# XiSHEN0220/RANSAC-Flow

Measured on NVIDIA H100. Metric: image-pairs/sec at 480x640, nbIter=1k RANSAC, higher is better.
Workload: dtype f32-grade: fp16 hi/lo split operands and activations (22 significand bits), 3 wgmma MMAs per MAC, fp32 accumulate; fp16-split correlation; fp32/fp64 RANSAC

## Files before the change

ransac-flow_b200/csrc/gemm_tc.cu:

```cuda
#include <cuda.h>
#include <cuda_fp16.h>

#include <climits>
#include <mutex>
#include <unordered_map>

#include "common.cuh"
#include "tc_common.cuh"

namespace rf {

constexpr int K_TF32 = 0, K_F16 = 1, K_SPLIT = 2, K_TF32X3 = 3;
constexpr int MODE_CONV = 0, MODE_CORR = 1;
constexpr int O_F32 = 0, O_F16 = 1, O_SPLIT = 2;
constexpr int WG_THREADS = 288;

struct alignas(64) WgParams {
    CUtensorMap mapA[RF_MAX_IMGS];
    CUtensorMap mapA2[RF_MAX_IMGS];
    CUtensorMap mapY[RF_MAX_IMGS];
    CUtensorMap mapR[RF_MAX_IMGS];
    CUtensorMap mapB;
    CUtensorMap mapBlo;
    int nimg;
    int ntiles;
    int tile_start[RF_MAX_IMGS + 1];
    int tiles_x[RF_MAX_IMGS];
    int tw[RF_MAX_IMGS];
    int Ho[RF_MAX_IMGS], Wo[RF_MAX_IMGS];
    long long out_pix[RF_MAX_IMGS + 1];
    int R, S, pad, stride, Cin, Cout, relu, round_out;
    int dil;
    int kc1, stride2;
    long long plane;
    const float* bias;
    const void* residual;
    void* y;
    unsigned long long* rowbest;
    unsigned long long* colbest;
    int NA, NB;
};
static_assert(sizeof(WgParams) <= 32764, "kernel parameter space (CUDA 12.1+ large kernel parameters)");

template <int KIND, int BN, int MODE>
struct WgCfg {
    static constexpr int NPL = (KIND == K_SPLIT || KIND == K_TF32X3) ? 2 : 1;
    static constexpr int A_BYTES = NPL * TC_A_BYTES;
    static constexpr int B_PLANE = BN * 128;
    static constexpr int STAGE_BYTES = A_BYTES + NPL * B_PLANE;
    static constexpr bool ONE_CTA = MODE == MODE_CORR || NPL * BN >= 256;
    static constexpr int BUDGET = ONE_CTA ? 200 * 1024 : 100 * 1024;
    static constexpr int STAGES = BUDGET / STAGE_BYTES > 6 ? 6 : BUDGET / STAGE_BYTES;
    static constexpr int CTAS_PER_SM = ONE_CTA ? 1 : 2;
    static constexpr int SMEM_BYTES = STAGES * STAGE_BYTES + 1024  + 256 ;
    static_assert(STAGES >= 2 && SMEM_BYTES <= 227 * 1024, "shared memory");
};

__device__ __forceinline__ __half2 pack_sat(float a, float b) {
    uint32_t r;
    asm("cvt.rn.satfinite.f16x2.f32 %0, %1, %2;" : "=r"(r) : "f"(b), "f"(a));
    return *reinterpret_cast<__half2*>(&r);
}
__device__ __forceinline__ void split2(float a, float b, __half2& hi, __half2& lo) {
    hi = pack_sat(a, b);
    const float2 f = __half22float2(hi);
    lo = pack_sat((a - f.x) * 2048.f, (b - f.y) * 2048.f);
}

template <int KIND, int BN, int NACC>
__device__ __forceinline__ void mma_block(float (&acc)[NACC][BN / 2], uint32_t sa, uint32_t sb) {
    constexpr bool TF32 = KIND == K_TF32 || KIND == K_TF32X3;
#pragma unroll
    for (int k = 0; k < 4; ++k) {
        const uint64_t ah = wg_desc(sa + 32 * k), bh = wg_desc(sb + 32 * k);
        if constexpr (KIND == K_SPLIT || KIND == K_TF32X3) {
            const uint64_t al = wg_desc(sa + TC_A_BYTES + 32 * k), bl = wg_desc(sb + BN * 128 + 32 * k);
            float (&x)[BN / 2] = acc[NACC - 1];
            wgmma<TF32, BN>(x, al, bh);
            wgmma<TF32, BN>(x, ah, bl);
            wgmma<TF32, BN>(acc[0], ah, bh);
        } else {
            wgmma<TF32, BN>(acc[0], ah, bh);
        }
    }
}

template <int KIND, int BN, int MODE, int OUT>
__global__ void __launch_bounds__(WG_THREADS, WgCfg<KIND, BN, MODE>::CTAS_PER_SM)
wg_kernel(const __grid_constant__ WgParams p) {
    using Cfg = WgCfg<KIND, BN, MODE>;
    constexpr int STAGES = Cfg::STAGES;
    constexpr int BK = (KIND == K_TF32 || KIND == K_TF32X3) ? TC_BK : TC_BK_F16;
    constexpr int NACC = KIND == K_SPLIT ? 2 : 1;
    constexpr bool SLOT = MODE == MODE_CONV && OUT != O_F32;
    constexpr int BOX_BYTES = (OUT == O_SPLIT ? 2 : 1) * 128 * 128;
    static_assert(!SLOT || (BN / 64) * BOX_BYTES <= Cfg::STAGE_BYTES, "the output tile fits one stage");
    extern __shared__ uint8_t smem_raw[];
    uint8_t* smem = smem_raw + ((1024u - (smem_u32(smem_raw) & 1023u)) & 1023u);
    uint64_t* full = reinterpret_cast<uint64_t*>(smem + STAGES * Cfg::STAGE_BYTES);
    uint64_t* empty = full + STAGES;
    const int warp = threadIdx.x >> 5, lane = threadIdx.x & 31;
    const int kc = p.Cin / BK;
    const int KI = p.R * p.S * kc;

    const int t_first = MODE == MODE_CORR ? 0 : (int)blockIdx.x;
    const int t_step = MODE == MODE_CORR ? 1 : (int)gridDim.x;
    const int t_end = MODE == MODE_CORR ? 1 : p.ntiles;
    const int nt = (p.Cout + BN - 1) / BN;
    struct Tile { int img, tw, ox0, oy0, n0; };
    auto decode = [&](int t) {
        const int mtile = MODE == MODE_CORR ? (int)blockIdx.y : t / nt;
        const int ntile = MODE == MODE_CORR ? (int)blockIdx.x : t - mtile * nt;
        Tile T;
        T.img = 0;
#pragma unroll
        for (int j = 1; j < RF_MAX_IMGS; ++j) T.img += (j < p.nimg && mtile >= p.tile_start[j]) ? 1 : 0;
        const int tloc = mtile - p.tile_start[T.img];
        T.tw = p.tw[T.img];
        const int tyi = tloc / p.tiles_x[T.img], txi = tloc - tyi * p.tiles_x[T.img];
        T.ox0 = txi * T.tw;
        T.oy0 = tyi * (128 / T.tw);
        T.n0 = ntile * BN;
        return T;
    };
    auto boxes = [&](const Tile& T) { return BN == 64 || T.n0 + 64 >= p.Cout ? 1 : 2; };

    if (threadIdx.x == 0) {
        for (int s = 0; s < STAGES; ++s) { mbar_init(&full[s], 1); mbar_init(&empty[s], 256); }
        fence_barrier_init();
    }
    __syncthreads();

    if (warp == 8) {
        if (lane == 0) {
            tma_prefetch_desc(&p.mapB);
            uint32_t prefetched = 0;
            int st = 0;
            uint32_t ph = 0;
            for (int t = t_first; t < t_end; t += t_step) {
                const Tile T = decode(t);
                if (!((prefetched >> T.img) & 1u)) {
                    prefetched |= 1u << T.img;
                    tma_prefetch_desc(&p.mapA[T.img]);
                    if constexpr (SLOT) {
                        tma_prefetch_desc(&p.mapY[T.img]);
                        if (p.residual) tma_prefetch_desc(&p.mapR[T.img]);
                    }
                }
                for (int it = 0; it < KI; ++it) {
                    mbar_wait(&empty[st], ph ^ 1);
                    uint8_t* sa = smem + st * Cfg::STAGE_BYTES;
                    uint8_t* sb = sa + Cfg::A_BYTES;
                    mbar_expect_tx(&full[st], Cfg::STAGE_BYTES);
                    if constexpr (MODE == MODE_CORR) {
                        const int c0 = it * BK;
                        tma_load_3d(sa, &p.mapA[0], &full[st], c0, T.ox0, 0);
                        tma_load_3d(sa + TC_A_BYTES, &p.mapA2[0], &full[st], c0, T.ox0, 0);
                        tma_load_2d(sb, &p.mapB, &full[st], c0, T.n0);
                        tma_load_2d(sb + Cfg::B_PLANE, &p.mapBlo, &full[st], c0, T.n0);
                    } else {
                        const int tap = it / kc, cc = it - tap * kc;
                        const int r = tap / p.S, s = tap - r * p.S;
                        const int c0 = cc * BK, x = T.ox0 * p.stride + s * p.dil - p.pad, y = T.oy0 * p.stride + r * p.dil - p.pad;
                        const int kcol = tap * p.Cin + c0;
                        if constexpr (KIND == K_SPLIT) {
                            if (cc < p.kc1) tma_load_4d(sa, &p.mapA[T.img], &full[st], c0, x, y, 0);
                            else tma_load_4d(sa, &p.mapA2[T.img], &full[st], (cc - p.kc1) * BK, T.ox0 * p.stride2, T.oy0 * p.stride2, 0);
                            tma_load_3d(sb, &p.mapB, &full[st], kcol, T.n0, 0);
                        } else {
                            tma_load_3d(sa, &p.mapA[T.img], &full[st], c0, x, y);
                            tma_load_2d(sb, &p.mapB, &full[st], kcol, T.n0);
                        }
                    }
                    if (++st == STAGES) { st = 0; ph ^= 1; }
                }
                if constexpr (SLOT) {
                    mbar_wait(&empty[st], ph ^ 1);
                    if (p.residual) {
// ... 6 lines not shown
                        }
                    } else {
                        mbar_arrive(&full[st]);
                    }
                    if (++st == STAGES) { st = 0; ph ^= 1; }
                }
            }
        }
        return;
    }

    const int g = warp >> 2;
    const int rbase = 64 * g + 16 * (warp & 3) + (lane >> 2);
    const int cbase = 2 * (lane & 3);
    auto before = [](int s) { return s == 0 ? STAGES - 1 : s - 1; };
    int st = 0;
    uint32_t ph = 0;
    bool stored = false;
    for (int t = t_first; t < t_end; t += t_step) {
        const Tile T = decode(t);
        float acc[NACC][BN / 2];
#pragma unroll
        for (int a = 0; a < NACC; ++a)
#pragma unroll
            for (int i = 0; i < BN / 2; ++i) acc[a][i] = 0.f;
        for (int it = 0; it < KI; ++it) {
            mbar_wait(&full[st], ph);
            const uint32_t sa = smem_u32(smem + st * Cfg::STAGE_BYTES);
            wg_fence();
            mma_block<KIND, BN, NACC>(acc, sa + g * (64 * 128), sa + Cfg::A_BYTES);
            wg_commit();
            wg_wait<1>();
            if (it > 0) {
                mbar_arrive(&empty[before(st)]);
            } else if (SLOT && stored) {
                if (threadIdx.x == 0) bulk_wait_read();
                mbar_arrive(&empty[before(st)]);
            }
            if (++st == STAGES) { st = 0; ph ^= 1; }
        }
        wg_wait<0>();
#pragma unroll
        for (int a = 0; a < NACC; ++a) wg_fence_regs(acc[a]);
        mbar_arrive(&empty[before(st)]);

        auto value = [&](int i) -> float {
            if constexpr (KIND == K_SPLIT) return fmaf(acc[1][i], 0.00048828125f, acc[0][i]);
            else return acc[0][i];
        };

        if constexpr (SLOT) {
            mbar_wait(&full[st], ph);
            uint8_t* slot = smem + st * Cfg::STAGE_BYTES;
#pragma unroll
            for (int h = 0; h < 2; ++h) {
                const int m = rbase + 8 * h;
#pragma unroll
                for (int j = 0; j < BN / 8; ++j) {
                    const int c = 8 * j + cbase, n = T.n0 + c;
                    if (n >= p.Cout) continue;
                    float v0 = value(4 * j + 2 * h), v1 = value(4 * j + 2 * h + 1);
                    if (p.bias) { v0 += __ldg(p.bias + n); v1 += __ldg(p.bias + n + 1); }
                    uint8_t* e = slot + (c >> 6) * BOX_BYTES + m * 128 + ((((c & 63) >> 3) ^ (m & 7)) << 4) + (c & 7) * 2;
                    if (p.residual) {
                        if constexpr (OUT == O_F16) {
                            const float2 r = __half22float2(*reinterpret_cast<const __half2*>(e));
                            v0 += r.x; v1 += r.y;
                        } else {
                            const float2 rh = __half22float2(*reinterpret_cast<const __half2*>(e));
                            const float2 rl = __half22float2(*reinterpret_cast<const __half2*>(e + 128 * 128));
                            v0 += fmaf(rl.x, 0.00048828125f, rh.x); v1 += fmaf(rl.y, 0.00048828125f, rh.y);
                        }
                    }
                    if (p.relu) { v0 = fmaxf(v0, 0.f); v1 = fmaxf(v1, 0.f); }
                    if constexpr (OUT == O_F16) {
                        *reinterpret_cast<__half2*>(e) = pack_sat(v0, v1);
                    } else {
                        __half2 hi, lo;
                        split2(v0, v1, hi, lo);
                        *reinterpret_cast<__half2*>(e) = hi;
                        *reinterpret_cast<__half2*>(e + 128 * 128) = lo;
                    }
                }
            }
            fence_proxy_async();
            asm volatile("bar.sync 1, 256;" ::: "memory");
            if (threadIdx.x == 0) {
                const int nb = boxes(T);
                for (int b = 0; b < nb; ++b) {
                    if constexpr (OUT == O_SPLIT) tma_store_4d(&p.mapY[T.img], slot + b * BOX_BYTES, T.n0 + 64 * b, T.ox0, T.oy0, 0);
                    else tma_store_3d(&p.mapY[T.img], slot + b * BOX_BYTES, T.n0 + 64 * b, T.ox0, T.oy0);
                }
                bulk_commit();
            }
            stored = true;
            if (++st == STAGES) { st = 0; ph ^= 1; }
        } else if constexpr (MODE == MODE_CONV) {
            const int img = T.img, tw = T.tw;
#pragma unroll
            for (int h = 0; h < 2; ++h) {
                const int m = rbase + 8 * h;
                const int py = m / tw, px = m - py * tw;
                const int oy = T.oy0 + py, ox = T.ox0 + px;
                if (oy >= p.Ho[img] || ox >= p.Wo[img]) continue;
                const long long pix = p.out_pix[img] + (long long)oy * p.Wo[img] + ox;
#pragma unroll
                for (int j = 0; j < BN / 8; ++j) {
                    const int n = T.n0 + 8 * j + cbase;
                    if (n >= p.Cout) continue;
                    const bool two = n + 1 < p.Cout;
                    float v0 = value(4 * j + 2 * h), v1 = value(4 * j + 2 * h + 1);
                    if (p.bias) { v0 += __ldg(p.bias + n); if (two) v1 += __ldg(p.bias + n + 1); }
                    const long long o = pix * p.Cout + n;
                    if (p.residual) {
                        const float* r = static_cast<const float*>(p.residual) + o;
                        v0 += __ldg(r); if (two) v1 += __ldg(r + 1);
                    }
                    if (p.relu) { v0 = fmaxf(v0, 0.f); v1 = fmaxf(v1, 0.f); }
                    if (p.round_out) { v0 = round_tf32(v0); v1 = round_tf32(v1); }
                    float* y = static_cast<float*>(p.y) + o;
                    if (two && (p.Cout & 1) == 0) *reinterpret_cast<float2*>(y) = make_float2(v0, v1);
                    else { y[0] = v0; if (two) y[1] = v1; }
                }
            }
        } else {
            const int n0 = T.n0;
            unsigned long long* sCol = reinterpret_cast<unsigned long long*>(smem);
            const int row0 = T.ox0 + rbase, row1 = row0 + 8;
            const bool rv0 = row0 < p.NA, rv1 = row1 < p.NA;
            unsigned long long rb0 = 0ull, rb1 = 0ull;
            asm volatile("bar.sync 1, 256;" ::: "memory");
#pragma unroll
            for (int j = 0; j < BN / 8; ++j) {
#pragma unroll
                for (int e = 0; e < 2; ++e) {
                    const int c = 8 * j + cbase + e, col = n0 + c;
                    const bool cv = col < p.NB;
                    const float s0 = value(4 * j + e), s1 = value(4 * j + 2 + e);
                    unsigned long long ck = 0ull;
                    if (cv) {
                        if (rv0) { const unsigned long long k = pack_key(s0, (uint32_t)col); rb0 = k > rb0 ? k : rb0; ck = pack_key(s0, (uint32_t)row0); }
                        if (rv1) { const unsigned long long k = pack_key(s1, (uint32_t)col); rb1 = k > rb1 ? k : rb1;
                                   const unsigned long long k1 = pack_key(s1, (uint32_t)row1); ck = k1 > ck ? k1 : ck; }
                    }
#pragma unroll
                    for (int off = 4; off < 32; off <<= 1) {
                        const unsigned long long o = __shfl_xor_sync(0xffffffffu, ck, off);
                        ck = o > ck ? o : ck;
                    }
                    if (lane < 4) sCol[warp * BN + c] = ck;
                }
            }
#pragma unroll
            for (int off = 1; off < 4; off <<= 1) {
                const unsigned long long o0 = __shfl_xor_sync(0xffffffffu, rb0, off), o1 = __shfl_xor_sync(0xffffffffu, rb1, off);
                rb0 = o0 > rb0 ? o0 : rb0;
                rb1 = o1 > rb1 ? o1 : rb1;
            }
            if ((lane & 3) == 0) {
                if (rv0 && rb0 != 0ull) atomicMax(p.rowbest + row0, rb0);
                if (rv1 && rb1 != 0ull) atomicMax(p.rowbest + row1, rb1);
            }
            asm volatile("bar.sync 1, 256;" ::: "memory");
            for (int c = threadIdx.x; c < BN; c += 256) {
                if (n0 + c >= p.NB) continue;
                unsigned long long cb = 0ull;
#pragma unroll
                for (int w = 0; w < 8; ++w) { const unsigned long long k = sCol[w * BN + c]; cb = k > cb ? k : cb; }
                if (cb != 0ull) atomicMax(p.colbest + n0 + c, cb);
            }
        }
    }
    if constexpr (SLOT)
        if (threadIdx.x == 0) bulk_wait();
}


constexpr int ST_TW = 32, ST_TH = 4, ST_C = 3;
constexpr int ST_PW = (ST_TW - 2) / 2, ST_PH = ST_TH / 2;
constexpr int ST_THREADS = 256;
constexpr int ST_B_PLANE = 64 * 128;
constexpr int ST_T_BYTES = 128 * 64 * 4;
static_assert(ST_PH * ST_PW * 8 <= ST_THREADS, "one thread per (pooled pixel, 8 channels) of a step");

template <int KS, int S>
struct StemGeo {
    static constexpr int PAD = (KS - 1) / 2;
    static constexpr int KK = KS * KS * ST_C;
    static constexpr int KSTEPS = (KK + 15) / 16;
    static constexpr int KB = (KSTEPS + 3) / 4;
    static constexpr int IN_H = (ST_TH - 1) * S + KS;
    static constexpr int IN_COLS = (ST_TW - 1) * S + KS;
    static constexpr int IN_W = IN_COLS * ST_C;
    static constexpr int EVEN_W = (IN_COLS + 1) / 2 * ST_C;
    static constexpr int LD = S == 2 ? 208 : 104;
    static constexpr int WIN = IN_H * LD;
    static constexpr int NLD = (IN_H * IN_W + ST_THREADS - 1) / ST_THREADS;
    static constexpr int NT = S == 2 ? 3 : 2;
    static constexpr int CTAS = S == 2 ? 1 : 2;
    static constexpr int OFF_T = KB * 2 * ST_B_PLANE;
    static constexpr int OFF_IN = OFF_T + NT * ST_T_BYTES;
    static constexpr int OFF_K = OFF_IN + 2 * WIN * 4;
    static constexpr int OFF_BAR = OFF_K + KSTEPS * 4 * 16;
    static constexpr int SMEM = OFF_BAR + 64 + 1024;
    static_assert(LD >= (S == 2 ? EVEN_W + IN_COLS / 2 * ST_C : IN_W), "window row");
    static_assert(CTAS * SMEM <= 227 * 1024, "stem shared memory");
    static __device__ __forceinline__ int word(int r, int ix, int c) { return r * LD + (S == 2 ? (ix & 1) * EVEN_W + (ix >> 1) * ST_C : ix * ST_C) + c; }
};

struct alignas(64) StemParams {
    CUtensorMap mapB;
    int nimg, pool;
    int unit_start[RF_MAX_IMGS + 1];
    int steps[RF_MAX_IMGS];
    int H[RF_MAX_IMGS], W[RF_MAX_IMGS];
    int Hs[RF_MAX_IMGS], Ws[RF_MAX_IMGS];
    int Ho[RF_MAX_IMGS], Wo[RF_MAX_IMGS];
    long long in_pix[RF_MAX_IMGS], out_pix[RF_MAX_IMGS];
    long long plane;
    const float* x;
    const float* bias;
    __half* y;
};

__device__ __forceinline__ uint32_t stem_pack_split(float v) {
    __half2 hi, lo;
    split2(v, 0.f, hi, lo);
    return (*reinterpret_cast<uint32_t*>(&hi) & 0xFFFFu) | (*reinterpret_cast<uint32_t*>(&lo) << 16);
}

struct StemFrag { uint32_t h[4], l[4]; };

template <int KK, int j>
__device__ __forceinline__ void stem_gather(StemFrag& f, const uint32_t* __restrict__ w, int base, const int4* sK, int q) {
    const int4 o4 = sK[j * 4 + q];
    const int o[4] = {o4.x, o4.y, o4.z, o4.w};
    uint32_t v[2][4];
#pragma unroll
    for (int h = 0; h < 2; ++h)
#pragma unroll
        for (int e = 0; e < 4; ++e) v[h][e] = (16 * (j + 1) <= KK || o[e] >= 0) ? w[base + 24 * h + o[e]] : 0u;
#pragma unroll
    for (int e = 0; e < 2; ++e)
#pragma unroll
        for (int h = 0; h < 2; ++h) {
            f.h[2 * e + h] = __byte_perm(v[h][2 * e], v[h][2 * e + 1], 0x5410);
            f.l[2 * e + h] = __byte_perm(v[h][2 * e], v[h][2 * e + 1], 0x7632);
        }
}

template <int KK, int KSTEPS, bool SPLIT, int j, int NACC>
__device__ __forceinline__ void stem_mma(float (&acc)[NACC][32], StemFrag (&buf)[2], const uint32_t* w, int base, const int4* sK, int q,
                                         uint32_t sB) {
    if constexpr (j < KSTEPS) {
        constexpr int NPL = SPLIT ? 2 : 1;
        StemFrag& f = buf[j & 1];
        wg_fence();
        const uint32_t b = sB + (j >> 2) * NPL * ST_B_PLANE + 32 * (j & 3);
        const uint64_t bh = wg_desc(b);
        if constexpr (SPLIT) {
            wgmma_f16_n64_rs(acc[1], f.l, bh);
            wgmma_f16_n64_rs(acc[1], f.h, wg_desc(b + ST_B_PLANE));
        }
        wgmma_f16_n64_rs(acc[0], f.h, bh);
        wg_commit();
        if constexpr (j + 1 < KSTEPS) {
            wg_wait<1>();
            stem_gather<KK, j + 1>(buf[(j + 1) & 1], w, base, sK, q);
        }
        stem_mma<KK, KSTEPS, SPLIT, j + 1>(acc, buf, w, base, sK, q, sB);
    }
}

template <int KS, int S, bool SPLIT>
__global__ void __launch_bounds__(ST_THREADS, StemGeo<KS, S>::CTAS)
stem_kernel(const __grid_constant__ StemParams p) {
    using G = StemGeo<KS, S>;
    constexpr int NPL = SPLIT ? 2 : 1;
    constexpr int NACC = SPLIT ? 2 : 1;
    constexpr int PIX_BYTES = SPLIT ? 256 : 128;
    extern __shared__ uint8_t smem_raw[];
    uint8_t* smem = smem_raw + ((1024u - (smem_u32(smem_raw) & 1023u)) & 1023u);
    uint8_t* sB = smem;
    uint8_t* sT = smem + G::OFF_T;
    uint32_t* sIn = reinterpret_cast<uint32_t*>(smem + G::OFF_IN);
    int4* sK = reinterpret_cast<int4*>(smem + G::OFF_K);
    uint64_t* bar_b = reinterpret_cast<uint64_t*>(smem + G::OFF_BAR);
    const int t = threadIdx.x, warp = t >> 5, lane = t & 31, g = warp >> 2;
    const long long units = p.unit_start[RF_MAX_IMGS];
    const int u_begin = (int)(units * blockIdx.x / gridDim.x), u_end = (int)(units * (blockIdx.x + 1) / gridDim.x);

    struct Unit { int img, strip, j, r0, c0; };
    auto decode = [&](int u) {
        Unit U;
        U.img = 0;
#pragma unroll
        for (int i = 1; i < RF_MAX_IMGS; ++i) U.img += (i < p.nimg && u >= p.unit_start[i]) ? 1 : 0;
        const int loc = u - p.unit_start[U.img];
        U.strip = loc / p.steps[U.img];
        U.j = loc - U.strip * p.steps[U.img];
        U.r0 = U.j * ST_TH;
        U.c0 = p.pool ? U.strip * 2 * ST_PW - 1 : U.strip * ST_TW;
        return U;
    };
    float win[G::NLD];
    auto load_window = [&](const Unit& U) {
        const int H = p.H[U.img], WC = p.W[U.img] * ST_C;
        const float* src = p.x + p.in_pix[U.img] * ST_C;
        const int iy0 = U.r0 * S - G::PAD, col0 = (U.c0 * S - G::PAD) * ST_C;
// ... 7 lines not shown
    };
    auto stage_window = [&](uint32_t* dst) {
#pragma unroll
        for (int i = 0; i < G::NLD; ++i) {
            const int idx = t + i * ST_THREADS;
            const int r = idx / G::IN_W, jj = idx - r * G::IN_W, ix = jj / ST_C;
            if (idx < G::IN_H * G::IN_W) dst[G::word(r, ix, jj - ix * ST_C)] = stem_pack_split(win[i]);
        }
    };

    if (t == 0) {
        mbar_init(bar_b, 1);
        fence_barrier_init();
    }
    if (t < G::KSTEPS * 4) {
        const int j = t >> 2, q = t & 3;
        int o[4];
#pragma unroll
        for (int e = 0; e < 4; ++e) {
            const int k = 16 * j + 2 * q + (e & 1) + 8 * (e >> 1);
            const int r = k / (KS * ST_C), rs = k - r * KS * ST_C, s = rs / ST_C;
            o[e] = k < G::KK ? G::word(r, s, rs - s * ST_C) : -1;
        }
        sK[t] = make_int4(o[0], o[1], o[2], o[3]);
    }
    __syncthreads();
    if (t == 0) {
        mbar_expect_tx(bar_b, G::KB * NPL * ST_B_PLANE);
#pragma unroll
        for (int kb = 0; kb < G::KB; ++kb) {
            if constexpr (SPLIT) tma_load_3d(sB + kb * 2 * ST_B_PLANE, &p.mapB, bar_b, kb * 64, 0, 0);
            else tma_load_2d(sB + kb * ST_B_PLANE, &p.mapB, bar_b, kb * 64, 0);
        }
    }
    int u = u_begin;
    Unit U = decode(u);
    if (p.pool && U.j > 0) U = decode(--u);
    load_window(U);
    stage_window(sIn);
    __syncthreads();

    const int q = lane & 3;
    const int rbase = 64 * g + 16 * (warp & 3) + (lane >> 2), cbase = 2 * q;
    const int base = (rbase >> 5) * S * G::LD + 3 * (rbase & 31);
    const uint32_t sB32 = smem_u32(sB);
    int wb = 0, tb = 0;
    for (bool first = true; u < u_end; ++u, first = false) {
        const uint32_t* w = sIn + wb * G::WIN;
        float acc[NACC][32];
#pragma unroll
        for (int a = 0; a < NACC; ++a)
#pragma unroll
            for (int i = 0; i < 32; ++i) acc[a][i] = 0.f;
        StemFrag frag[2];
        stem_gather<G::KK, 0>(frag[0], w, base, sK, q);
        if (first) mbar_wait(bar_b, 0);
        stem_mma<G::KK, G::KSTEPS, SPLIT, 0>(acc, frag, w, base, sK, q, sB32);
        const bool more = u + 1 < u_end;
        Unit N = U;
        if (more) {
            N = decode(u + 1);
            load_window(N);
        }
        wg_wait<0>();
#pragma unroll
        for (int a = 0; a < NACC; ++a) wg_fence_regs(acc[a]);

        const int img = U.img;
        uint8_t* tile = sT + tb * ST_T_BYTES;
#pragma unroll
        for (int h = 0; h < 2; ++h) {
            const int mm = rbase + 8 * h;
#pragma unroll
            for (int j = 0; j < 8; ++j) {
                const int n = 8 * j + cbase, i = 4 * j + 2 * h;
                float v0 = SPLIT ? fmaf(acc[NACC - 1][i], 0.00048828125f, acc[0][i]) : acc[0][i];
                float v1 = SPLIT ? fmaf(acc[NACC - 1][i + 1], 0.00048828125f, acc[0][i + 1]) : acc[0][i + 1];
                if (p.bias) { v0 += __ldg(p.bias + n); v1 += __ldg(p.bias + n + 1); }
                v0 = fmaxf(v0, 0.f);
                v1 = fmaxf(v1, 0.f);
                uint8_t* e = tile + mm * 128 + ((j ^ (mm & 7)) << 4) + cbase * 2;
                if constexpr (SPLIT) {
                    __half2 hi, lo;
                    split2(v0, v1, hi, lo);
                    if (p.pool) {
                        const float2 fh = __half22float2(hi), fl = __half22float2(lo);
                        *reinterpret_cast<float2*>(tile + mm * PIX_BYTES + (((n >> 2) ^ (mm & 7)) << 4) + (n & 3) * 4) =
                            make_float2(fmaf(fl.x, 0.00048828125f, fh.x), fmaf(fl.y, 0.00048828125f, fh.y));
                    } else {
                        *reinterpret_cast<__half2*>(e) = hi;
                        *reinterpret_cast<__half2*>(e + 128 * 128) = lo;
                    }
                } else {
                    *reinterpret_cast<__half2*>(e) = pack_sat(v0, v1);
                }
            }
        }
        if (more) stage_window(sIn + (wb ^ 1) * G::WIN);
        __syncthreads();

        if (!p.pool) {
            for (int i = t; i < NPL * 128 * 8; i += ST_THREADS) {
                const int pl = i >> 10, mm = (i >> 3) & 127, ch = i & 7;
                const int oy = U.r0 + (mm >> 5), ox = U.c0 + (mm & 31);
                if (oy < p.Ho[img] && ox < p.Wo[img])
                    *reinterpret_cast<uint4*>(p.y + pl * p.plane + (p.out_pix[img] + (long long)oy * p.Wo[img] + ox) * 64 + ch * 8) =
                        *reinterpret_cast<const uint4*>(tile + pl * 128 * 128 + mm * 128 + ((ch ^ (mm & 7)) << 4));
// ... 132 lines not shown
    CUresult r = enc(out, esize == 2 ? CU_TENSOR_MAP_DATA_TYPE_FLOAT16 : CU_TENSOR_MAP_DATA_TYPE_FLOAT32, rank, const_cast<void*>(ptr), dims, strides, box, es,
                     CU_TENSOR_MAP_INTERLEAVE_NONE, CU_TENSOR_MAP_SWIZZLE_128B, CU_TENSOR_MAP_L2_PROMOTION_L2_256B,
                     CU_TENSOR_MAP_FLOAT_OOB_FILL_NONE);
    if (r != CUDA_SUCCESS) {
        snprintf(g_err, sizeof(g_err), "cuTensorMapEncodeTiled failed with CUresult %d (dims %llu,%llu,%llu,%llu box %u,%u,%u,%u)", (int)r, d0, d1, d2, d3, b0, b1, b2, b3);
        return 3;
    }
    if (g_maps.size() > 8192) g_maps.clear();
    g_maps[key] = *out;
    return 0;
}

int get_map(CUtensorMap* out, const void* ptr, unsigned long long d0, unsigned long long d1, unsigned long long d2,
            unsigned b0, unsigned b1, unsigned b2, unsigned es_, unsigned esize) {
    return get_map4(out, ptr, d0, d1, d2, 0, 0, b0, b1, b2, 0, es_, esize);
}

int pick_tw(int Ho, int Wo) {
    int best = 16;
    long long best_area = -1;
    const int cands[5] = {16, 32, 8, 64, 128};
    for (int i = 0; i < 5; ++i) {
        int tw = cands[i], th = 128 / tw;
        long long area = (long long)((Wo + tw - 1) / tw) * ((Ho + th - 1) / th);
        if (best_area < 0 || area < best_area) { best_area = area; best = tw; }
    }
    return best;
}

template <int KIND, int BN, int MODE, int OUT>
static int launch_wg(const WgParams& p, dim3 grid, cudaStream_t st) {
    using Cfg = WgCfg<KIND, BN, MODE>;
    static bool attr[64] = {false};
    const int dev = current_device();
    if (!attr[dev]) {
        RF_CUDA(cudaFuncSetAttribute(wg_kernel<KIND, BN, MODE, OUT>, cudaFuncAttributeMaxDynamicSharedMemorySize, Cfg::SMEM_BYTES));
        attr[dev] = true;
    }
    wg_kernel<KIND, BN, MODE, OUT><<<grid, WG_THREADS, Cfg::SMEM_BYTES, st>>>(p);
    RF_LAUNCHED();
    return 0;
}

template <int KIND, int BN, int OUT>
static int launch_conv_bn(const WgParams& p, cudaStream_t st) {
    const int resident = WgCfg<KIND, BN, MODE_CONV>::CTAS_PER_SM * num_sms();
    return launch_wg<KIND, BN, MODE_CONV, OUT>(p, dim3(p.ntiles < resident ? p.ntiles : resident), st);
}
template <int KIND, int OUT>
static int launch_conv(const WgParams& p, int BN, cudaStream_t st) {
    return BN == 128 ? launch_conv_bn<KIND, 128, OUT>(p, st) : launch_conv_bn<KIND, 64, OUT>(p, st);
}

struct SplitDual { const void* x2; const int* hw2; int Cin2, stride2; };

static int conv_impl(const ImgSet& batch, const ConvParams& cp, const void* w, cudaStream_t st, int kind, bool out32, const SplitDual* dual) {
    const bool flat = cp.R == 1 && cp.S == 1 && cp.stride == 1 && cp.pad == 0 && (dual == nullptr || dual->stride2 == 1);
    int hw_flat[2] = {1, 0};
    ImgSet flat_set;
    if (flat) {
        RF_REQUIRE(batch.out_pix[batch.n] <= INT_MAX, "rf_conv2d_nhwc: more than 2^31 - 1 pixels in one batch");
        hw_flat[1] = (int)batch.out_pix[batch.n];
        RF_REQUIRE(make_imgset(flat_set, 1, hw_flat, 1, 1, 0) == 0, "rf_conv2d_nhwc: bad image set");
    }
    const ImgSet& set = flat ? flat_set : batch;
    const int* hw2 = dual == nullptr ? nullptr : flat ? hw_flat : dual->hw2;
    WgParams p;
    memset(&p, 0, sizeof(p));
    const bool split = kind == K_SPLIT;
    const unsigned esz = kind == K_TF32 ? 4u : 2u;
    const unsigned bk = kind == K_TF32 ? TC_BK : TC_BK_F16;
    const int BN = cp.Cout > 64 ? 128 : 64;
    const char* xb = reinterpret_cast<const char*>(cp.x);
    const unsigned long long in_plane = (unsigned long long)set.in_pix[set.n] * cp.Cin * 2ull;
    long long in2_pix[RF_MAX_IMGS + 1] = {0};
    if (dual)
        for (int i = 0; i < set.n; ++i) in2_pix[i + 1] = in2_pix[i] + (long long)hw2[2 * i] * hw2[2 * i + 1];
    const unsigned long long in2_plane = dual ? (unsigned long long)in2_pix[set.n] * dual->Cin2 * 2ull : 0ull;
    p.nimg = set.n;
    const bool tma_out = kind != K_TF32 && !out32;
    const unsigned long long out_plane = (unsigned long long)set.out_pix[set.n] * cp.Cout * 2ull;
    const char* yb = reinterpret_cast<const char*>(cp.y);
    const char* rb = reinterpret_cast<const char*>(cp.residual);
    int tiles = 0;
    for (int i = 0; i < set.n; ++i) {
        const int tw = flat ? 128 : pick_tw(set.Ho[i], set.Wo[i]), th = 128 / tw;
        p.tw[i] = tw;
        p.tiles_x[i] = (set.Wo[i] + tw - 1) / tw;
        p.tile_start[i] = tiles;
        tiles += p.tiles_x[i] * ((set.Ho[i] + th - 1) / th);
        p.Ho[i] = set.Ho[i]; p.Wo[i] = set.Wo[i];
        p.out_pix[i] = set.out_pix[i];
        int rc = split ? get_map4(&p.mapA[i], xb + set.in_pix[i] * cp.Cin * 2, (unsigned long long)cp.Cin, (unsigned long long)set.W[i],
                                  (unsigned long long)set.H[i], 2, in_plane, bk, (unsigned)tw, (unsigned)th, 2, (unsigned)cp.stride, 2)
                       : get_map(&p.mapA[i], xb + set.in_pix[i] * cp.Cin * esz, (unsigned long long)cp.Cin, (unsigned long long)set.W[i],
                                 (unsigned long long)set.H[i], bk, (unsigned)tw, (unsigned)th, (unsigned)cp.stride, esz);
        if (!rc && dual)
            rc = get_map4(&p.mapA2[i], static_cast<const char*>(dual->x2) + in2_pix[i] * dual->Cin2 * 2, (unsigned long long)dual->Cin2,
                          (unsigned long long)hw2[2 * i + 1], (unsigned long long)hw2[2 * i], 2, in2_plane, bk, (unsigned)tw,
                          (unsigned)th, 2, (unsigned)dual->stride2, 2);
        const long long o = set.out_pix[i] * cp.Cout * 2;
        for (int m = 0; m < (cp.residual ? 2 : 1) && tma_out && !rc; ++m) {
            CUtensorMap* map = m == 0 ? &p.mapY[i] : &p.mapR[i];
            const void* base = (m == 0 ? yb : rb) + o;
            rc = split ? get_map4(map, base, (unsigned long long)cp.Cout, (unsigned long long)set.Wo[i], (unsigned long long)set.Ho[i], 2,
                                  out_plane, 64, (unsigned)tw, (unsigned)th, 2, 1, 2)
                       : get_map(map, base, (unsigned long long)cp.Cout, (unsigned long long)set.Wo[i], (unsigned long long)set.Ho[i],
                                 64, (unsigned)tw, (unsigned)th, 1, 2);
        }
        if (rc) return rc;
    }
    RF_REQUIRE(tiles > 0, "rf_conv2d_nhwc: empty output");
    for (int i = set.n; i <= RF_MAX_IMGS; ++i) p.tile_start[i] = tiles;
    p.out_pix[set.n] = set.out_pix[set.n];
    int rc = split ? get_map(&p.mapB, w, (unsigned long long)cp.K, (unsigned long long)cp.Cout, 2, bk, (unsigned)BN, 2, 1, 2)
                   : get_map(&p.mapB, w, (unsigned long long)cp.K, (unsigned long long)cp.Cout, 0, bk, (unsigned)BN, 0, 1, esz);
    if (rc) return rc;
    p.R = cp.R; p.S = cp.S; p.pad = cp.pad; p.stride = cp.stride; p.Cin = cp.Cin; p.Cout = cp.Cout; p.relu = cp.relu; p.round_out = cp.round_out;
    p.dil = cp.dil;
    p.kc1 = cp.Cin / (int)bk;
    p.stride2 = 1;
    if (dual) { p.Cin = cp.Cin + dual->Cin2; p.stride2 = dual->stride2; }
    p.plane = (long long)set.out_pix[set.n] * cp.Cout;
    p.bias = cp.bias; p.residual = cp.residual; p.y = cp.y;
    p.ntiles = tiles * ((cp.Cout + BN - 1) / BN);
    if (kind == K_TF32) return launch_conv<K_TF32, O_F32>(p, BN, st);
    if (kind == K_F16) return out32 ? launch_conv<K_F16, O_F32>(p, BN, st) : launch_conv<K_F16, O_F16>(p, BN, st);
    return out32 ? launch_conv<K_SPLIT, O_F32>(p, BN, st) : launch_conv<K_SPLIT, O_SPLIT>(p, BN, st);
}

template <int KS, int S, bool SPLIT>
static int stem_impl(const float* x, int nimg, const int* hw_host, const void* w, const float* bias, void* y, int pool, void* stream) {
    using G = StemGeo<KS, S>;
    RF_REQUIRE(x != nullptr && w != nullptr && y != nullptr, "rf_stem: null pointer");
    RF_REQUIRE(((uintptr_t)y % 16) == 0 && ((uintptr_t)w % 16) == 0, "rf_stem: pointers must be 16-byte aligned");
    ImgSet set;
    RF_REQUIRE(make_imgset(set, nimg, hw_host, KS, S, G::PAD) == 0, "rf_stem: bad image set");
    StemParams p;
    memset(&p, 0, sizeof(p));
    p.nimg = nimg;
    p.pool = pool ? 1 : 0;
    int units = 0;
    long long out = 0;
    for (int i = 0; i < nimg; ++i) {
        const int Hs = set.Ho[i], Ws = set.Wo[i];
        const int Ho = pool ? (Hs - 1) / 2 + 1 : Hs, Wo = pool ? (Ws - 1) / 2 + 1 : Ws;
        const int strips = pool ? (Wo + ST_PW - 1) / ST_PW : (Ws + ST_TW - 1) / ST_TW;
        p.steps[i] = pool ? (Ho + ST_PH - 1) / ST_PH : (Hs + ST_TH - 1) / ST_TH;
        p.unit_start[i] = units;
        units += strips * p.steps[i];
        p.H[i] = set.H[i]; p.W[i] = set.W[i]; p.Hs[i] = Hs; p.Ws[i] = Ws; p.Ho[i] = Ho; p.Wo[i] = Wo;
        p.in_pix[i] = set.in_pix[i];
        p.out_pix[i] = out;
        out += (long long)Ho * Wo;
    }
    for (int i = nimg; i <= RF_MAX_IMGS; ++i) p.unit_start[i] = units;
    constexpr unsigned long long K = G::KB * 64ull;
    int rc = SPLIT ? get_map(&p.mapB, w, K, 64ull, 2, 64, 64, 2, 1, 2) : get_map(&p.mapB, w, K, 64ull, 0, 64, 64, 0, 1, 2);
    if (rc) return rc;
    p.plane = out * 64;
    p.x = x; p.bias = bias; p.y = static_cast<__half*>(y);
    static bool attr[64] = {false};
    const int dev = current_device();
    if (!attr[dev]) {
        RF_CUDA(cudaFuncSetAttribute(stem_kernel<KS, S, SPLIT>, cudaFuncAttributeMaxDynamicSharedMemorySize, G::SMEM));
        attr[dev] = true;
    }
    const int resident = G::CTAS * num_sms();
    stem_kernel<KS, S, SPLIT><<<units < resident ? units : resident, ST_THREADS, G::SMEM, as_stream(stream)>>>(p);
    RF_LAUNCHED();
    return 0;
}

}

using namespace rf;

bool rf_conv2d_tc_supported(const ConvParams& p) {
// ... 120 lines not shown
```

Before: 158.5.

## Add halo-tile 3x3 conv kernel that reuses one input halo across all taps

Adds a dedicated kernel for 3x3 stride-1 split-fp16 convolutions with 64 or 128 input channels and BN=64. Each output tile loads its input halo once via TMA and feeds all nine taps from shared memory with ldmatrix register-sourced wgmma. The old path re-fetched a shifted A tile per tap. The kernel also double-buffers halos across tiles and prefetches the residual into the output slot. The epilogue is factored into shared helpers. The cost is a more complex producer/consumer barrier scheme and different shared-memory budgeting and occupancy.

```diff
diff --git a/ransac-flow_b200/csrc/gemm_tc.cu b/ransac-flow_b200/csrc/gemm_tc.cu
--- a/ransac-flow_b200/csrc/gemm_tc.cu
+++ b/ransac-flow_b200/csrc/gemm_tc.cu
@@ -39,6 +39,7 @@
     unsigned long long* rowbest;
     unsigned long long* colbest;
     int NA, NB;
+    int nhalo, halo_slot, bstages;
 };
 static_assert(sizeof(WgParams) <= 32764, "kernel parameter space (CUDA 12.1+ large kernel parameters)");
 
@@ -85,6 +86,81 @@
     }
 }
 
+struct Tile { int img, tw, ox0, oy0, n0; };
+__device__ __forceinline__ Tile pixel_tile(const WgParams& p, int mtile, int n0) {
+    Tile T;
+    T.img = 0;
+#pragma unroll
+    for (int j = 1; j < RF_MAX_IMGS; ++j) T.img += (j < p.nimg && mtile >= p.tile_start[j]) ? 1 : 0;
+    const int tloc = mtile - p.tile_start[T.img];
+    T.tw = p.tw[T.img];
+    const int tyi = tloc / p.tiles_x[T.img], txi = tloc - tyi * p.tiles_x[T.img];
+    T.ox0 = txi * T.tw;
+    T.oy0 = tyi * (128 / T.tw);
+    T.n0 = n0;
+    return T;
+}
+template <int BN>
+__device__ __forceinline__ int out_boxes(const WgParams& p, const Tile& T) { return BN == 64 || T.n0 + 64 >= p.Cout ? 1 : 2; }
+
+template <int OUT>
+constexpr int slot_box_bytes() { return (OUT == O_SPLIT ? 2 : 1) * 128 * 128; }
+
+template <int KIND, int BN, int OUT, int NACC>
+__device__ __forceinline__ void slot_epilogue(float (&acc)[NACC][BN / 2], uint8_t* slot, const WgParams& p, int n0, int rbase, int cbase) {
+    constexpr int BOX_BYTES = slot_box_bytes<OUT>();
+    auto value = [&](int i) -> float {
+        if constexpr (KIND == K_SPLIT) return fmaf(acc[1][i], 0.00048828125f, acc[0][i]);
+        else return acc[0][i];
+    };
+#pragma unroll
+    for (int h = 0; h < 2; ++h) {
+        const int m = rbase + 8 * h;
+#pragma unroll
+        for (int j = 0; j < BN / 8; ++j) {
+            const int c = 8 * j + cbase, n = n0 + c;
+            if (n >= p.Cout) continue;
+            float v0 = value(4 * j + 2 * h), v1 = value(4 * j + 2 * h + 1);
+            if (p.bias) { v0 += __ldg(p.bias + n); v1 += __ldg(p.bias + n + 1); }
+            uint8_t* e = slot + (c >> 6) * BOX_BYTES + m * 128 + ((((c & 63) >> 3) ^ (m & 7)) << 4) + (c & 7) * 2;
+            if (p.residual) {
+                if constexpr (OUT == O_F16) {
+                    const float2 r = __half22float2(*reinterpret_cast<const __half2*>(e));
+                    v0 += r.x; v1 += r.y;
+                } else {
+                    const float2 rh = __half22float2(*reinterpret_cast<const __half2*>(e));
+                    const float2 rl = __half22float2(*reinterpret_cast<const __half2*>(e + 128 * 128));
+                    v0 += fmaf(rl.x, 0.00048828125f, rh.x); v1 += fmaf(rl.y, 0.00048828125f, rh.y);
+                }
+            }
+            if (p.relu) { v0 = fmaxf(v0, 0.f); v1 = fmaxf(v1, 0.f); }
+            if constexpr (OUT == O_F16) {
+                *reinterpret_cast<__half2*>(e) = pack_sat(v0, v1);
+            } else {
+                __half2 hi, lo;
+                split2(v0, v1, hi, lo);
+                *reinterpret_cast<__half2*>(e) = hi;
+                *reinterpret_cast<__half2*>(e + 128 * 128) = lo;
+            }
+        }
+    }
+}
+
+template <int BN, int OUT>
+__device__ __forceinline__ void slot_store(const WgParams& p, const uint8_t* slot, const Tile& T) {
+    constexpr int BOX_BYTES = slot_box_bytes<OUT>();
+    fence_proxy_async();
+    asm volatile("bar.sync 1, 256;" ::: "memory");
+    if (threadIdx.x == 0) {
+        const int nb = out_boxes<BN>(p, T);
+        for (int b = 0; b < nb; ++b) {
+            if constexpr (OUT == O_SPLIT) tma_store_4d(&p.mapY[T.img], slot + b * BOX_BYTES, T.n0 + 64 * b, T.ox0, T.oy0, 0);
+            else tma_store_3d(&p.mapY[T.img], slot + b * BOX_BYTES, T.n0 + 64 * b, T.ox0, T.oy0);
+        }
+        bulk_commit();
+    }
+}
+
 template <int KIND, int BN, int MODE, int OUT>
 __global__ void __launch_bounds__(WG_THREADS, WgCfg<KIND, BN, MODE>::CTAS_PER_SM)
 wg_kernel(const __grid_constant__ WgParams p) {
@@ -93,7 +169,7 @@
     constexpr int BK = (KIND == K_TF32 || KIND == K_TF32X3) ? TC_BK : TC_BK_F16;
     constexpr int NACC = KIND == K_SPLIT ? 2 : 1;
     constexpr bool SLOT = MODE == MODE_CONV && OUT != O_F32;
-    constexpr int BOX_BYTES = (OUT == O_SPLIT ? 2 : 1) * 128 * 128;
+    constexpr int BOX_BYTES = slot_box_bytes<OUT>();
     static_assert(!SLOT || (BN / 64) * BOX_BYTES <= Cfg::STAGE_BYTES, "the output tile fits one stage");
     extern __shared__ uint8_t smem_raw[];
     uint8_t* smem = smem_raw + ((1024u - (smem_u32(smem_raw) & 1023u)) & 1023u);
@@ -107,23 +183,12 @@
     const int t_step = MODE == MODE_CORR ? 1 : (int)gridDim.x;
     const int t_end = MODE == MODE_CORR ? 1 : p.ntiles;
     const int nt = (p.Cout + BN - 1) / BN;
-    struct Tile { int img, tw, ox0, oy0, n0; };
     auto decode = [&](int t) {
         const int mtile = MODE == MODE_CORR ? (int)blockIdx.y : t / nt;
         const int ntile = MODE == MODE_CORR ? (int)blockIdx.x : t - mtile * nt;
-        Tile T;
-        T.img = 0;
-#pragma unroll
-        for (int j = 1; j < RF_MAX_IMGS; ++j) T.img += (j < p.nimg && mtile >= p.tile_start[j]) ? 1 : 0;
-        const int tloc = mtile - p.tile_start[T.img];
-        T.tw = p.tw[T.img];
-        const int tyi = tloc / p.tiles_x[T.img], txi = tloc - tyi * p.tiles_x[T.img];
-        T.ox0 = txi * T.tw;
-        T.oy0 = tyi * (128 / T.tw);
-        T.n0 = ntile * BN;
-        return T;
+        return pixel_tile(p, mtile, ntile * BN);
     };
-    auto boxes = [&](const Tile& T) { return BN == 64 || T.n0 + 64 >= p.Cout ? 1 : 2; };
+    auto boxes = [&](const Tile& T) { return out_boxes<BN>(p, T); };
 
     if (threadIdx.x == 0) {
         for (int s = 0; s < STAGES; ++s) { mbar_init(&full[s], 1); mbar_init(&empty[s], 256); }
@@ -236,47 +301,8 @@
         if constexpr (SLOT) {
             mbar_wait(&full[st], ph);
             uint8_t* slot = smem + st * Cfg::STAGE_BYTES;
-#pragma unroll
-            for (int h = 0; h < 2; ++h) {
-                const int m = rbase + 8 * h;
-#pragma unroll
-                for (int j = 0; j < BN / 8; ++j) {
-                    const int c = 8 * j + cbase, n = T.n0 + c;
-                    if (n >= p.Cout) continue;
-                    float v0 = value(4 * j + 2 * h), v1 = value(4 * j + 2 * h + 1);
-                    if (p.bias) { v0 += __ldg(p.bias + n); v1 += __ldg(p.bias + n + 1); }
-                    uint8_t* e = slot + (c >> 6) * BOX_BYTES + m * 128 + ((((c & 63) >> 3) ^ (m & 7)) << 4) + (c & 7) * 2;
-                    if (p.residual) {
-                        if constexpr (OUT == O_F16) {
-                            const float2 r = __half22float2(*reinterpret_cast<const __half2*>(e));
-                            v0 += r.x; v1 += r.y;
-                        } else {
-                            const float2 rh = __half22float2(*reinterpret_cast<const __half2*>(e));
-                            const float2 rl = __half22float2(*reinterpret_cast<const __half2*>(e + 128 * 128));
-                            v0 += fmaf(rl.x, 0.00048828125f, rh.x); v1 += fmaf(rl.y, 0.00048828125f, rh.y);
-                        }
-                    }
-                    if (p.relu) { v0 = fmaxf(v0, 0.f); v1 = fmaxf(v1, 0.f); }
-                    if constexpr (OUT == O_F16) {
-                        *reinterpret_cast<__half2*>(e) = pack_sat(v0, v1);
-                    } else {
-                        __half2 hi, lo;
-                        split2(v0, v1, hi, lo);
-                        *reinterpret_cast<__half2*>(e) = hi;
-                        *reinterpret_cast<__half2*>(e + 128 * 128) = lo;
-                    }
-                }
-            }
-            fence_proxy_async();
-            asm volatile("bar.sync 1, 256;" ::: "memory");
-            if (threadIdx.x == 0) {
-                const int nb = boxes(T);
-                for (int b = 0; b < nb; ++b) {
-                    if constexpr (OUT == O_SPLIT) tma_store_4d(&p.mapY[T.img], slot + b * BOX_BYTES, T.n0 + 64 * b, T.ox0, T.oy0, 0);
-                    else tma_store_3d(&p.mapY[T.img], slot + b * BOX_BYTES, T.n0 + 64 * b, T.ox0, T.oy0);
-                }
-                bulk_commit();
-            }
+            slot_epilogue<KIND, BN, OUT, NACC>(acc, slot, p, T.n0, rbase, cbase);
+            slot_store<BN, OUT>(p, slot, T);
             stored = true;
             if (++st == STAGES) { st = 0; ph ^= 1; }
         } else if constexpr (MODE == MODE_CONV) {
@@ -359,6 +385,175 @@
         if (threadIdx.x == 0) bulk_wait();
 }
 
+__host__ __device__ constexpr int halo_cb_bytes(int tw) { return ((tw + 2) * (128 / tw + 2) * 256 + 1023) & ~1023; }
+
+struct SplitFrag { uint32_t h[4], l[4]; };
+
+__device__ __forceinline__ void ldsm_x4(uint32_t (&r)[4], uint32_t addr) {
+    asm volatile("ldmatrix.sync.aligned.m8n8.x4.shared.b16 {%0, %1, %2, %3}, [%4];"
+                 : "=r"(r[0]), "=r"(r[1]), "=r"(r[2]), "=r"(r[3]) : "r"(addr) : "memory");
+}
+
+__device__ __forceinline__ void halo_frag(SplitFrag& f, uint32_t cb, int hr, int rows, int k, int half) {
+    const int c = 2 * k + half;
+    const int lh = hr, ll = hr + rows;
+    ldsm_x4(f.h, cb + lh * 128 + ((c ^ (lh & 7)) << 4));
+    ldsm_x4(f.l, cb + ll * 128 + ((c ^ (ll & 7)) << 4));
+}
+
+constexpr int HALO_MAX_BSTAGES = 6;
+
+constexpr int HALO_THREADS = 256;
+
+template <int KC>
+__global__ void __launch_bounds__(HALO_THREADS, 2)
+halo3_kernel(const __grid_constant__ WgParams p) {
+    constexpr int BN = 64;
+    constexpr int B_STAGE = 2 * BN * 128;
+    constexpr int KI = 9 * KC;
+    constexpr int BOX_BYTES = slot_box_bytes<O_SPLIT>();
+    extern __shared__ uint8_t smem_raw[];
+    uint8_t* smem = smem_raw + ((1024u - (smem_u32(smem_raw) & 1023u)) & 1023u);
+    const int NH = p.nhalo, BST = p.bstages;
+    uint8_t* slot = smem + NH * p.halo_slot;
+    uint8_t* sB = slot + BOX_BYTES;
+    uint64_t* bfull = reinterpret_cast<uint64_t*>(sB + BST * B_STAGE);
+    uint64_t* bempty = bfull + HALO_MAX_BSTAGES;
+    uint64_t* hfull = bempty + HALO_MAX_BSTAGES;
+    uint64_t* hempty = hfull + 2;
+    uint64_t* ofull = hempty + 2;
+    const int warp = threadIdx.x >> 5, lane = threadIdx.x & 31;
+    const bool producer = threadIdx.x == 0;
+    const int nt = (p.Cout + BN - 1) / BN;
+    auto decode = [&](int t) { const int mtile = t / nt; return pixel_tile(p, mtile, (t - mtile * nt) * BN); };
+
+    int pt = blockIdx.x, pit = 0, pbs = 0;
+    uint32_t pph = 0;
+    auto load_b = [&]() {
+        if (pt >= p.ntiles) return;
+        mbar_wait(&bempty[pbs], pph ^ 1);
+        mbar_expect_tx(&bfull[pbs], B_STAGE);
+        const int tap = pit / KC, cb = pit - tap * KC, mtile = pt / nt;
+        tma_load_3d(sB + pbs * B_STAGE, &p.mapB, &bfull[pbs], tap * p.Cin + 64 * cb, (pt - mtile * nt) * BN, 0);
+        if (++pit == KI) { pit = 0; pt += gridDim.x; }
+        if (++pbs == BST) { pbs = 0; pph ^= 1; }
+    };
+    auto load_halo = [&](int t, int u) {
+        const Tile T = decode(t);
+        const int h = u % NH;
+        mbar_wait(&hempty[h], ((uint32_t)(u / NH) & 1u) ^ 1u);
+        mbar_expect_tx(&hfull[h], KC * (T.tw + 2) * (128 / T.tw + 2) * 256);
+#pragma unroll
+        for (int cb = 0; cb < KC; ++cb)
+            tma_load_4d(smem + h * p.halo_slot + cb * halo_cb_bytes(T.tw), &p.mapA[T.img], &hfull[h], 64 * cb, T.ox0 - 1, T.oy0 - 1, 0);
+    };
+    auto load_slot = [&](const Tile& T) {
+        if (p.residual) {
+            mbar_expect_tx(ofull, BOX_BYTES);
+            tma_load_4d(slot, &p.mapR[T.img], ofull, T.n0, T.ox0, T.oy0, 0);
+        } else {
+            mbar_arrive(ofull);
+        }
+    };
+
+    if (producer) {
+        for (int s = 0; s < BST; ++s) { mbar_init(&bfull[s], 1); mbar_init(&bempty[s], HALO_THREADS); }
+        for (int h = 0; h < NH; ++h) { mbar_init(&hfull[h], 1); mbar_init(&hempty[h], HALO_THREADS); }
+        mbar_init(ofull, 1);
+        fence_barrier_init();
+        tma_prefetch_desc(&p.mapB);
+        for (int i = 0; i < p.nimg; ++i) {
+            tma_prefetch_desc(&p.mapA[i]);
+            tma_prefetch_desc(&p.mapY[i]);
+            if (p.residual) tma_prefetch_desc(&p.mapR[i]);
+        }
+        if (blockIdx.x < p.ntiles) {
+            load_halo(blockIdx.x, 0);
+            load_slot(decode(blockIdx.x));
+        }
+        for (int s = 0; s < BST; ++s) load_b();
+    }
+    __syncthreads();
+
+    const int g = warp >> 2;
+    const int rbase = 64 * g + 16 * (warp & 3) + (lane >> 2);
+    const int cbase = 2 * (lane & 3);
+    const int arow = 64 * g + 16 * (warp & 3) + (lane & 15);
+    const int half = lane >> 4;
+    int bs = 0, bprev = 0;
+    uint32_t bph = 0;
+    int u = 0;
+    for (int t = blockIdx.x; t < p.ntiles; t += gridDim.x, ++u) {
+        const Tile T = decode(t);
+        const int h = u % NH;
+        const bool next = t + (int)gridDim.x < p.ntiles;
+        if (producer && NH == 2 && next) load_halo(t + gridDim.x, u + 1);
+        const uint32_t halo32 = smem_u32(smem + h * p.halo_slot);
+        const int hw = T.tw + 2, rows = hw * (128 / T.tw + 2), cbb = halo_cb_bytes(T.tw);
+        const int py = arow / T.tw, px = arow - py * T.tw;
+        const int hr0 = py * hw + px;
+        float acc[2][BN / 2];
+#pragma unroll
+        for (int a = 0; a < 2; ++a)
+#pragma unroll
+            for (int i = 0; i < BN / 2; ++i) acc[a][i] = 0.f;
+        auto at = [&](int it, uint32_t& cb32, int& hr) {
+            const int tap = it / KC, cb = it - tap * KC, r = tap / 3;
+            cb32 = halo32 + cb * cbb;
+            hr = hr0 + r * hw + tap - 3 * r;
+        };
+        mbar_wait(&hfull[h], (uint32_t)(u / NH) & 1u);
+        SplitFrag f[2];
+        uint32_t cb32;
+        int hr;
+        at(0, cb32, hr);
+        halo_frag(f[0], cb32, hr, rows, 0, half);
+        for (int it = 0; it < KI; ++it) {
+            mbar_wait(&bfull[bs], bph);
+            const uint32_t sb = smem_u32(sB + bs * B_STAGE);
+#pragma unroll
+            for (int k = 0; k < 4; ++k) {
+                wg_fence();
+                const uint64_t bh = wg_desc(sb + 32 * k), bl = wg_desc(sb + BN * 128 + 32 * k);
+                wgmma_f16_n64_rs(acc[1], f[k & 1].l, bh);
+                wgmma_f16_n64_rs(acc[1], f[k & 1].h, bl);
+                wgmma_f16_n64_rs(acc[0], f[k & 1].h, bh);
+                wg_commit();
+                wg_wait<1>();
+                if (k == 0 && it > 0) {
+                    mbar_arrive(&bempty[bprev]);
+                    if (producer) load_b();
+                }
+                if (k == 0 && it == 0 && u > 0 && producer) {
+                    bulk_wait_read();
+                    load_slot(T);
+                }
+                if (k == 3) {
+                    if (it + 1 == KI) break;
+                    at(it + 1, cb32, hr);
+                }
+                halo_frag(f[(k + 1) & 1], cb32, hr, rows, (k + 1) & 3, half);
+            }
+            bprev = bs;
+            if (++bs == BST) { bs = 0; bph ^= 1; }
+        }
+        wg_wait<0>();
+#pragma unroll
+        for (int a = 0; a < 2; ++a) wg_fence_regs(acc[a]);
+        mbar_arrive(&bempty[bprev]);
+        mbar_arrive(&hempty[h]);
+        if (producer) {
+            load_b();
+            if (NH == 1 && next) load_halo(t + gridDim.x, u + 1);
+        }
+
+        mbar_wait(ofull, u & 1);
+        slot_epilogue<K_SPLIT, BN, O_SPLIT, 2>(acc, slot, p, T.n0, rbase, cbase);
+        slot_store<BN, O_SPLIT>(p, slot, T);
+    }
+    if (producer) bulk_wait();
+}
+
 
 constexpr int ST_TW = 32, ST_TH = 4, ST_C = 3;
 constexpr int ST_PW = (ST_TW - 2) / 2, ST_PH = ST_TH / 2;
@@ -413,10 +608,8 @@
     return (*reinterpret_cast<uint32_t*>(&hi) & 0xFFFFu) | (*reinterpret_cast<uint32_t*>(&lo) << 16);
 }
 
-struct StemFrag { uint32_t h[4], l[4]; };
-
 template <int KK, int j>
-__device__ __forceinline__ void stem_gather(StemFrag& f, const uint32_t* __restrict__ w, int base, const int4* sK, int q) {
+__device__ __forceinline__ void stem_gather(SplitFrag& f, const uint32_t* __restrict__ w, int base, const int4* sK, int q) {
     const int4 o4 = sK[j * 4 + q];
     const int o[4] = {o4.x, o4.y, o4.z, o4.w};
     uint32_t v[2][4];
@@ -434,11 +627,11 @@
 }
 
 template <int KK, int KSTEPS, bool SPLIT, int j, int NACC>
-__device__ __forceinline__ void stem_mma(float (&acc)[NACC][32], StemFrag (&buf)[2], const uint32_t* w, int base, const int4* sK, int q,
+__device__ __forceinline__ void stem_mma(float (&acc)[NACC][32], SplitFrag (&buf)[2], const uint32_t* w, int base, const int4* sK, int q,
                                          uint32_t sB) {
     if constexpr (j < KSTEPS) {
         constexpr int NPL = SPLIT ? 2 : 1;
-        StemFrag& f = buf[j & 1];
+        SplitFrag& f = buf[j & 1];
         wg_fence();
         const uint32_t b = sB + (j >> 2) * NPL * ST_B_PLANE + 32 * (j & 3);
         const uint64_t bh = wg_desc(b);
@@ -552,7 +745,7 @@
         for (int a = 0; a < NACC; ++a)
 #pragma unroll
             for (int i = 0; i < 32; ++i) acc[a][i] = 0.f;
-        StemFrag frag[2];
+        SplitFrag frag[2];
         stem_gather<G::KK, 0>(frag[0], w, base, sK, q);
         if (first) mbar_wait(bar_b, 0);
         stem_mma<G::KK, G::KSTEPS, SPLIT, 0>(acc, frag, w, base, sK, q, sB32);
@@ -791,6 +984,36 @@
     return BN == 128 ? launch_conv_bn<KIND, 128, OUT>(p, st) : launch_conv_bn<KIND, 64, OUT>(p, st);
 }
 
+static int halo_plan(WgParams& p, int halo, int& ctas) {
+    constexpr int stage = 2 * 64 * 128, out = slot_box_bytes<O_SPLIT>(), fixed = 1024  + 256 ;
+    p.halo_slot = halo;
+    p.nhalo = 1;
+    ctas = 2;
+    int budget = 113 * 1024 - fixed;
+    if (halo + out + 2 * stage > budget) {
+        ctas = 1;
+        budget = 227 * 1024 - fixed;
+        p.nhalo = 2 * halo + out + 2 * stage <= budget ? 2 : 1;
+    }
+    const int st = (budget - p.nhalo * halo - out) / stage;
+    p.bstages = st > HALO_MAX_BSTAGES ? HALO_MAX_BSTAGES : st;
+    return p.bstages >= 2 ? p.nhalo * halo + out + p.bstages * stage + fixed : 0;
+}
+
+template <int KC>
+static int launch_halo3(const WgParams& p, int smem, int ctas, cudaStream_t st) {
+    static bool attr[64] = {false};
+    const int dev = current_device();
+    if (!attr[dev]) {
+        RF_CUDA(cudaFuncSetAttribute(halo3_kernel<KC>, cudaFuncAttributeMaxDynamicSharedMemorySize, 227 * 1024));
+        attr[dev] = true;
+    }
+    const int resident = ctas * num_sms();
+    halo3_kernel<KC><<<p.ntiles < resident ? p.ntiles : resident, HALO_THREADS, smem, st>>>(p);
+    RF_LAUNCHED();
+    return 0;
+}
+
 struct SplitDual { const void* x2; const int* hw2; int Cin2, stride2; };
 
 static int conv_impl(const ImgSet& batch, const ConvParams& cp, const void* w, cudaStream_t st, int kind, bool out32, const SplitDual* dual) {
@@ -821,6 +1044,16 @@
     const unsigned long long out_plane = (unsigned long long)set.out_pix[set.n] * cp.Cout * 2ull;
     const char* yb = reinterpret_cast<const char*>(cp.y);
     const char* rb = reinterpret_cast<const char*>(cp.residual);
+    int halo_smem = 0, halo_ctas = 0;
+    if (split && !out32 && dual == nullptr && cp.R == 3 && cp.S == 3 && cp.stride == 1 && cp.pad == 1 && cp.dil == 1 &&
+        (cp.Cin == 64 || cp.Cin == 128) && BN == 64) {
+        int halo = 0;
+        for (int i = 0; i < set.n; ++i) {
+            const int b = (cp.Cin / 64) * halo_cb_bytes(pick_tw(set.Ho[i], set.Wo[i]));
+            halo = b > halo ? b : halo;
+        }
+        halo_smem = halo_plan(p, halo, halo_ctas);
+    }
     int tiles = 0;
     for (int i = 0; i < set.n; ++i) {
         const int tw = flat ? 128 : pick_tw(set.Ho[i], set.Wo[i]), th = 128 / tw;
@@ -830,8 +1063,9 @@
         tiles += p.tiles_x[i] * ((set.Ho[i] + th - 1) / th);
         p.Ho[i] = set.Ho[i]; p.Wo[i] = set.Wo[i];
         p.out_pix[i] = set.out_pix[i];
+        const unsigned ab1 = halo_smem ? tw + 2 : tw, ab2 = halo_smem ? th + 2 : th;
         int rc = split ? get_map4(&p.mapA[i], xb + set.in_pix[i] * cp.Cin * 2, (unsigned long long)cp.Cin, (unsigned long long)set.W[i],
-                                  (unsigned long long)set.H[i], 2, in_plane, bk, (unsigned)tw, (unsigned)th, 2, (unsigned)cp.stride, 2)
+                                  (unsigned long long)set.H[i], 2, in_plane, bk, ab1, ab2, 2, (unsigned)cp.stride, 2)
                        : get_map(&p.mapA[i], xb + set.in_pix[i] * cp.Cin * esz, (unsigned long long)cp.Cin, (unsigned long long)set.W[i],
                                  (unsigned long long)set.H[i], bk, (unsigned)tw, (unsigned)th, (unsigned)cp.stride, esz);
         if (!rc && dual)
@@ -863,6 +1097,9 @@
     p.plane = (long long)set.out_pix[set.n] * cp.Cout;
     p.bias = cp.bias; p.residual = cp.residual; p.y = cp.y;
     p.ntiles = tiles * ((cp.Cout + BN - 1) / BN);
+    if (halo_smem) {
+        return cp.Cin == 64 ? launch_halo3<1>(p, halo_smem, halo_ctas, st) : launch_halo3<2>(p, halo_smem, halo_ctas, st);
+    }
     if (kind == K_TF32) return launch_conv<K_TF32, O_F32>(p, BN, st);
     if (kind == K_F16) return out32 ? launch_conv<K_F16, O_F32>(p, BN, st) : launch_conv<K_F16, O_F16>(p, BN, st);
     return out32 ? launch_conv<K_SPLIT, O_F32>(p, BN, st) : launch_conv<K_SPLIT, O_SPLIT>(p, BN, st);
```

After: 161.2, median of 6. 1.02x the previous value.
